# sina-behnam/RTSDS

Measured on AMD Instinct MI355X. Metric: images/sec/node (train step) + inference FPS@1024x512, BiSeNet 19-cls, higher is better.
Workload: dtype bf16; 1 GPU; configs[1]: BiSeNet-R18 seg-only train step (train.py:65-113); model=BiSeNet-ResNet18, global_batch=8, per_gpu_batch=8, image=3x512x1024, num_classes=19, parallelism=dp1

## Files before the change

include/rtsds_hip.h:

```cpp
#ifndef RTSDS_HIP_H
#define RTSDS_HIP_H
#include <stddef.h>
#include <stdint.h>
#ifdef __cplusplus
extern "C" {
#endif

enum { RTSDS_F32 = 0, RTSDS_BF16 = 1, RTSDS_F16 = 2  };
enum {
  RTSDS_OK = 0,
  RTSDS_ERR_SHAPE = 1,
  RTSDS_ERR_UNSUPPORTED = 2,
  RTSDS_ERR_LAUNCH = 3,
  RTSDS_ERR_WORKSPACE = 4
};
enum { RTSDS_ACT_NONE = 0, RTSDS_ACT_RELU = 1, RTSDS_ACT_LEAKY = 2, RTSDS_ACT_SIGMOID = 3 };
#define RTSDS_ACCUMULATE 0x100
#define RTSDS_INPUT_PADDED 0x400
#define RTSDS_WEIGHT_PACKED 0x800

typedef struct {
  int n, h, w, c;
  int ho, wo, k;
  int kh, kw;
// ... 188 lines not shown
int rtsds_ce_weighted_bwd(const void* x, long sn, long sc, long shw, const int64_t* target,
                          const float* weight, const float* grad_loss, const float* count, void* dx,
                          int n, long hw, int c, int ignore_index, int dtype, void* stream);
int rtsds_bce_fwd(const float* x, const float* target, float* loss, int n, void* stream);
int rtsds_bce_bwd(const float* x, const float* target, const float* grad_loss, float* dx, int n,
                  void* stream);

int rtsds_adam_step(float* param, const void* grad, float* exp_avg, float* exp_avg_sq,
                    void* bf16_shadow, long n, float lr, float beta1, float beta2, float eps,
                    float weight_decay, int step, float grad_scale, int grad_dtype, void* stream);

int rtsds_adam_step_dev(float* param, const void* grad, float* exp_avg, float* exp_avg_sq,
                        void* bf16_shadow, long n, const float* hyper, float beta1, float beta2,
                        float eps, float weight_decay, float grad_scale, int grad_dtype, void* stream);

int rtsds_sgd_step(float* param, const void* grad, float* momentum_buf, void* bf16_shadow,
                   long n, const float* hyper, float lr, float momentum, float dampening,
                   float weight_decay, int nesterov, int first, float grad_scale, int grad_dtype, void* stream);

int rtsds_ema_step(float* teacher, const float* student, void* teacher_bf16_shadow, long n, float w,
                   void* stream);
int rtsds_ema_many(int count, float* const* teacher, const float* const* student, const long* numel,
                   float w, void* stream);

int rtsds_argmax(const void* x, long sn, long sc, long shw, int64_t* out, const int64_t* target,
                 unsigned long long* correct, int n, long hw, int c, int dtype, void* stream);
int rtsds_confusion(const int64_t* label, const int64_t* pred, unsigned long long* hist, long total,
                    int nc, void* stream);

#define RTSDS_UPCE_SET_CORRECT 2
// ... 126 lines not shown
                        void* pooled, void* hid, void* att, void* r, int ldr, int n, long hw, int c, int dtype,
                        void* stream);
int rtsds_ffm_att_bwd(const void* dr, const void* f, const void* a, const void* h, const void* p, const void* w1,
                      const void* w2, float* dw1, float* db1, float* dw2, float* db2, void* dp, int n, long hw, int c,
                      int accumulate, int dtype, void* ws, size_t ws_bytes, void* stream);
int rtsds_bn_bwd_ffm(const void* dr, const void* att, const void* dpooled, int n, long hw, const void* x, void* dx,
                     float* dgamma, float* dbeta, int c, const float* gamma, const float* beta, const float* save_mean,
                     const float* save_invstd, int training, int act, int accumulate_params, int dtype, void* ws,
                     size_t ws_bytes, void* stream);

size_t rtsds_label_stats_workspace(int n, int c);
int rtsds_label_stats(const int64_t* label, int n, int h, int w, int c, int ignore_index,
                      unsigned long long* count, unsigned long long* support, void* ws, size_t ws_bytes,
                      void* stream);

#define RTSDS_ABI_VERSION 28
int rtsds_abi_version(void);

#ifdef __cplusplus
}
#endif
#endif
```

rtsds_amd/_lib.py:

```python
import ctypes
import os

import torch

_HERE = os.path.dirname(os.path.abspath(__file__))
DEFAULT_LIB_PATH = os.path.join(_HERE, "librtsds_hip.so")
ABI_VERSION = 28
LIB_PATH = os.environ.get("RTSDS_LIB") or DEFAULT_LIB_PATH

F32, BF16 = 0, 1
ACT_NONE, ACT_RELU, ACT_LEAKY, ACT_SIGMOID = 0, 1, 2, 3
ACCUMULATE = 0x100
INPUT_PADDED = 0x400
WEIGHT_PACKED = 0x800
UPCE_SET_CORRECT = 2
ERRORS = {1: "bad shape", 2: "unsupported configuration", 3: "HIP launch failure", 4: "workspace too small"}

c_int, c_long, c_float, c_double, c_size_t, c_void_p = (ctypes.c_int, ctypes.c_long, ctypes.c_float, ctypes.c_double,
                                                        ctypes.c_size_t, ctypes.c_void_p)


class ConvDesc(ctypes.Structure):
    _fields_ = [(n, c_int) for n in ("n", "h", "w", "c", "ho", "wo", "k", "kh", "kw", "sh", "sw",
                                     "ph", "pw", "dh", "dw", "dtype")]
# ... 102 lines not shown
    "rtsds_softmax_fwd": (c_int, [P, c_long, c_long, c_long, P, c_int, c_int, c_long, c_int, c_int, P]),
    "rtsds_softmax_bwd": (c_int, [P, P, c_int, P, c_long, c_long, c_long, c_int, c_long, c_int, c_int,
                                  P]),
    "rtsds_ce_workspace": (c_size_t, []),
    "rtsds_ce_fwd": (c_int, [P, c_long, c_long, c_long, P, P, c_int, c_long, c_int, c_int, c_int, P,
                             c_size_t, P]),
    "rtsds_ce_bwd": (c_int, [P, c_long, c_long, c_long, P, P, P, P, c_int, c_long, c_int, c_int, c_int,
                             P]),
    "rtsds_ce_weighted_fwd": (c_int, [P, c_long, c_long, c_long, P, P, P, c_int, c_long, c_int, c_int, c_int, P,
                                      c_size_t, P]),
    "rtsds_ce_weighted_bwd": (c_int, [P, c_long, c_long, c_long, P, P, P, P, P, c_int, c_long, c_int, c_int, c_int,
                                      P]),
    "rtsds_bce_fwd": (c_int, [P, P, P, c_int, P]),
    "rtsds_bce_bwd": (c_int, [P, P, P, P, c_int, P]),
    "rtsds_adam_step_dev": (c_int, [P, P, P, P, P, c_long, P, c_float, c_float, c_float, c_float, c_float, c_int, P]),
    "rtsds_upsoftmax_fwd": (c_int, [P, P, c_int, c_int, c_int, c_int, c_int, c_int, c_float, c_float, c_int, c_int, P]),
    "rtsds_upsoftmax_bwd_workspace": (c_size_t, [c_int, c_int, c_int, c_int, c_int, c_int]),
    "rtsds_upsoftmax_bwd": (c_int, [P, c_int, P, c_int, P, c_int, c_int, c_int, c_int, c_int, c_int, c_float, c_float,
                                    c_int, P, c_size_t, P]),
    "rtsds_upselfinfo_fwd": (c_int, [P, P, c_int, c_int, c_int, c_int, c_int, c_int, c_float, c_float, c_int, c_int, P]),
    "rtsds_upselfinfo_bwd_workspace": (c_size_t, [c_int, c_int, c_int, c_int, c_int, c_int]),
    "rtsds_upselfinfo_bwd": (c_int, [P, c_int, P, P, c_int, c_int, c_int, c_int, c_int, c_int, c_float, c_float, c_int, P,
                                     c_size_t, P]),
    "rtsds_upsoftmax_acc": (c_int, [P, P, P, c_int, c_int, c_int, c_int, c_int, c_int, c_float, c_float, c_int, c_int,
                                    c_int, P]),
    "rtsds_conf_hist": (c_int, [P, P, P, P, c_long, c_int, c_int, c_float, P]),
    "rtsds_pseudo_select": (c_int, [P, P, P, P, c_long, c_int, c_int, P]),
    "rtsds_upsample_pseudo": (c_int, [P, P, P, P, P] + [c_int] * 6 + [c_float, c_float, c_int, c_int, c_int, P]),
    "rtsds_upsample_paint": (c_int, [P, P, P, P, P, P] + [c_int] * 6 + [c_float, c_float, c_int, c_int, P]),
    "rtsds_slide_paint": (c_int, [P, ctypes.POINTER(c_int), c_int, P, P, P, P, P, P] + [c_int] * 8 +
# ... 88 lines not shown
```

rtsds_amd/csrc/conv_wgrad.hip:

```cpp
#include "conv_host.h"

template <int V>
__global__ void __launch_bounds__(256) split_reduce_kernel(const float* __restrict__ part, float* __restrict__ out, int nv,
                                                            int cv, FastDiv fcv, int cp, long slab, int splits, int accumulate) {
  __shared__ float red[4][64][V];
  const int lane = threadIdx.x & 63, sg = threadIdx.x >> 6;
  for (int i0 = blockIdx.x * 64; i0 < nv; i0 += gridDim.x * 64) {
    const int i = i0 + lane;
    const bool ok = i < nv;
    const int rt = (int)fdiv((uint32_t)(ok ? i : 0), fcv);
    const long src = (long)rt * cp + (long)((ok ? i : 0) - rt * cv) * V;
    float s[V];
#pragma unroll
    for (int e = 0; e < V; ++e) s[e] = 0.f;
    for (int q = sg; ok && q < splits; q += 32) {
      float t[8][V];
#pragma unroll
      for (int u = 0; u < 8; ++u) {
        const long off = (long)min(q + 4 * u, splits - 1) * slab + src;
        if constexpr (V == 4) {
          const f32x4 v = *(const f32x4*)(part + off);
#pragma unroll
          for (int e = 0; e < V; ++e) t[u][e] = v[e];
        } else {
// ... 203 lines not shown

static const int kReduceBatch = 16;
struct ReduceBatch {
  rtsds_split_reduce_desc d[kReduceBatch];
  int blk0[kReduceBatch];
  int n;
};
__global__ void __launch_bounds__(256) split_reduce_many_kernel(const ReduceBatch b) {
  __shared__ float red[4][64][4];
  int si = 0;
  for (int i = 1; i < b.n; ++i)
    if (b.blk0[i] <= (int)blockIdx.x) si = i;
  const rtsds_split_reduce_desc& q = b.d[si];
  const int lane = threadIdx.x & 63, sg = threadIdx.x >> 6;
  const int i = ((int)blockIdx.x - b.blk0[si]) * 64 + lane;
  const bool ok = i < q.nv;
  const int rt = (ok ? i : 0) / q.cv;
  const long src = (long)rt * q.cp + (long)((ok ? i : 0) - rt * q.cv) * 4;
  float s[4] = {0.f, 0.f, 0.f, 0.f};
  for (int g = sg; ok && g < q.splits; g += 32) {
    float t[8][4];
#pragma unroll
    for (int u = 0; u < 8; ++u) {
      const f32x4 v = *(const f32x4*)(q.slab + (long)min(g + 4 * u, q.splits - 1) * q.slab_stride + src);
#pragma unroll
      for (int e = 0; e < 4; ++e) t[u][e] = v[e];
    }
#pragma unroll
    for (int u = 0; u < 8; ++u)
      if (g + 4 * u < q.splits)
#pragma unroll
        for (int e = 0; e < 4; ++e) s[e] += t[u][e];
  }
#pragma unroll
  for (int e = 0; e < 4; ++e) red[sg][lane][e] = s[e];
  __syncthreads();
  if (sg == 0 && ok) {
    float* o = q.dw + (long)i * 4;
#pragma unroll
    for (int e = 0; e < 4; ++e) {
      const float t = (red[0][lane][e] + red[1][lane][e]) + (red[2][lane][e] + red[3][lane][e]);
      o[e] = q.accumulate ? o[e] + t : t;
    }
  }
}
extern "C" int rtsds_split_reduce_many(int n, const rtsds_split_reduce_desc* descs, void* stream) {
  if (n < 0 || (n && !descs)) return RTSDS_ERR_SHAPE;
  for (int i0 = 0; i0 < n; i0 += kReduceBatch) {
    ReduceBatch b;
    b.n = 0;
    int blocks = 0;
    for (int i = i0; i < n && b.n < kReduceBatch; ++i) {
      if (descs[i].nv <= 0) continue;
      if (descs[i].cv <= 0 || descs[i].splits <= 0 || !descs[i].slab || !descs[i].dw) return RTSDS_ERR_SHAPE;
      b.d[b.n] = descs[i];
      b.blk0[b.n] = blocks;
      blocks += (descs[i].nv + 63) / 64;
      ++b.n;
// ... 192 lines not shown
```

rtsds_amd/csrc/optim.hip:

```cpp
#include "ew_common.h"

template <typename GT>
__global__ void adam_kernel(float* __restrict__ p, const GT* __restrict__ g, float* __restrict__ m, float* __restrict__ v,
                            bf16* __restrict__ shadow, long n, float lr, float b1, float b2, float eps, float wd, float bc1,
                            float bc2_sqrt, float gscale) {
  const float step = lr / bc1;
  GRID_STRIDE(i, n) {
    float gi = to_f(g[i]) * gscale;
    float pi = p[i];
    if (wd != 0.f) gi = fmaf(wd, pi, gi);
    float mi = m[i], vi = v[i];
    mi = fmaf(1.f - b1, gi - mi, mi);
    vi = fmaf(b2, vi, (1.f - b2) * gi * gi);
    const float den = sqrtf(vi) / bc2_sqrt + eps;
    pi -= step * (mi / den);
    m[i] = mi;
    v[i] = vi;
    p[i] = pi;
    if (shadow) shadow[i] = (bf16)pi;
  }
}
template <typename GT>
__global__ void adam_dev_kernel(float* __restrict__ p, const GT* __restrict__ g, float* __restrict__ m, float* __restrict__ v,
                                bf16* __restrict__ shadow, long n, const float* __restrict__ hyper, float b1, float b2, float eps,
                                float wd, float gscale) {
  const float lr = hyper[0], bc1 = hyper[1], bc2_sqrt = hyper[2];
  const float step = lr / bc1;
  GRID_STRIDE(i, n) {
    float gi = to_f(g[i]) * gscale;
    float pi = p[i];
    if (wd != 0.f) gi = fmaf(wd, pi, gi);
    float mi = m[i], vi = v[i];
    mi = fmaf(1.f - b1, gi - mi, mi);
    vi = fmaf(b2, vi, (1.f - b2) * gi * gi);
    const float den = sqrtf(vi) / bc2_sqrt + eps;
    pi -= step * (mi / den);
    m[i] = mi;
    v[i] = vi;
    p[i] = pi;
    if (shadow) shadow[i] = (bf16)pi;
  }
}
#define DISPATCH_GRAD(gd, ...)                                               \
  do {                                                                       \
    if ((gd) == RTSDS_F32) { typedef float GT; __VA_ARGS__; }                \
    else if ((gd) == RTSDS_BF16) { typedef bf16 GT; __VA_ARGS__; }           \
    else if ((gd) == RTSDS_F16) { typedef f16 GT; __VA_ARGS__; }             \
    else return RTSDS_ERR_UNSUPPORTED;                                       \
  } while (0)
extern "C" int rtsds_adam_step_dev(float* param, const void* grad, float* exp_avg, float* exp_avg_sq, void* bf16_shadow,
                                   long n, const float* hyper, float beta1, float beta2, float eps, float weight_decay,
                                   float grad_scale, int grad_dtype, void* stream) {
  if (n <= 0 || !hyper) return RTSDS_ERR_SHAPE;
  DISPATCH_GRAD(grad_dtype, hipLaunchKernelGGL(adam_dev_kernel<GT>, dim3(ew_blocks(n, 256, 4096)), dim3(256), 0,
                                               (hipStream_t)stream, param, (const GT*)grad, exp_avg, exp_avg_sq,
                                               (bf16*)bf16_shadow, n, hyper, beta1, beta2, eps, weight_decay, grad_scale));
  RET_LAUNCH();
}

extern "C" int rtsds_adam_step(float* param, const void* grad, float* exp_avg, float* exp_avg_sq, void* bf16_shadow, long n, float lr,
                               float beta1, float beta2, float eps, float weight_decay, int step, float grad_scale, int grad_dtype,
                               void* stream) {
  if (n <= 0 || step <= 0) return RTSDS_ERR_SHAPE;
  const double bc1 = 1.0 - pow((double)beta1, step), bc2 = 1.0 - pow((double)beta2, step);
  DISPATCH_GRAD(grad_dtype, hipLaunchKernelGGL(adam_kernel<GT>, dim3(ew_blocks(n, 256, 4096)), dim3(256), 0, (hipStream_t)stream,
                                               param, (const GT*)grad, exp_avg, exp_avg_sq, (bf16*)bf16_shadow, n, lr, beta1, beta2,
                                               eps, weight_decay, (float)bc1, (float)sqrt(bc2), grad_scale));
  RET_LAUNCH();
}

template <typename GT>
__global__ void sgd_kernel(float* __restrict__ p, const GT* __restrict__ g, float* __restrict__ buf,
                           bf16* __restrict__ shadow, long n, const float* __restrict__ hyper, float lr, float momentum,
                           float dampening, float wd, int nesterov, int first, float gscale) {
// ... 95 lines not shown
```

rtsds_amd/functional.py:

```python
import ctypes

import numpy as np
import torch

from ._lib import (ACT_RELU, ACT_SIGMOID, INPUT_PADDED, UPCE_SET_CORRECT, WEIGHT_PACKED, BnParams, ConvDesc,
                   SplitReduceDesc, lib)
from .runtime import (CL, bump_params_epoch, collective, dcode, dp_world, empty_nhwc, nhwc, params_epoch,
                      register_fold, require_hip, side_enabled, side_fork, stream, workspace)

_P = lambda t: None if t is None else t.data_ptr()

CONV_PROFILE = None


def _conv_flops(d):
    return 2.0 * d.n * d.ho * d.wo * d.k * d.c * d.kh * d.kw


class _Timed:
    def __init__(self, d, tag="fwd"):
        self.d, self.tag = d, tag

    def __enter__(self):
        if CONV_PROFILE is not None:
# ... 124 lines not shown


def _join_add(join, g):
    if join is None:
        return g
    if join.buf is not None:
        if join.first:
            join.buf.add_(g)
            return join.put(join.buf)
        g.add_(join.buf)
    return join.put(g)


DEFER_WGRAD_REDUCE = True
_deferred = []


def flush_wgrad_reduce():
    global _deferred
    items, _deferred = _deferred, []
    if not items:
        return
    cur = torch.cuda.current_stream(items[0][1].device)
    for st in {it[2] for it in items}:
        if st != cur:
            cur.wait_stream(st)
    batch, seen = [], set()
    for desc, _ws, _st in items + [(None, None, None)]:
        if desc is None or desc.dw in seen or len(batch) == 16:
            if batch:
                arr = (SplitReduceDesc * len(batch))(*batch)
                lib.rtsds_split_reduce_many(len(batch), arr, cur.cuda_stream)
            batch, seen = [], set()
        if desc is not None:
            batch.append(desc)
            seen.add(desc.dw)
    for _desc, ws, st in items:
        if st != cur:
            ws.record_stream(cur)


def _wgrad_into_arena(d, x, g, sinks, xflag, ws):
    if DEFER_WGRAD_REDUCE and CONV_PROFILE is None and x.dtype == torch.bfloat16:
        pend = SplitReduceDesc()
        lib.rtsds_conv2d_wgrad_deferred(ctypes.byref(d), _P(x), _P(g), _P(sinks[0]), _P(sinks[1]), 1 | xflag,
                                        _P(ws), ws.numel(), ctypes.byref(pend), stream())
        if pend.nv > 0:
            _deferred.append((pend, ws, torch.cuda.current_stream(ws.device)))
            torch.autograd.Variable._execution_engine.queue_callback(flush_wgrad_reduce)
        return
    with _Timed(d, "wgrad"):
        lib.rtsds_conv2d_wgrad(ctypes.byref(d), _P(x), _P(g), _P(sinks[0]), _P(sinks[1]), 1 | xflag,
                               _P(ws), ws.numel(), stream())


class ConvFn(torch.autograd.Function):

    @staticmethod
    def forward(ctx, x, weight, bias, wq, stride, padding, dilation, act, stats, join=None, fold=(0, False),
                bn_link=None, wg_link=None):
        require_hip(x, weight)
        k, _, kh, kw = weight.shape
        padded = hasattr(x, "_rt_cpad") and is_padded_input(x, _conv_desc(x, k, kh, kw, stride, padding, dilation))
        if not padded:
# ... 69 lines not shown
                                                   _P(bsm), _P(bsi), bact | wpk, _P(part), _P(ws), ws.numel(), stream())
                    link.part, link.nrb = part, tiles
                elif ctx.in_act:
                    lib.rtsds_conv2d_dgrad_act(ctypes.byref(d), _P(g), _P(wd), _P(dx), _P(x), ctx.in_act | wpk,
                                               _P(ws), ws.numel(), stream())
                else:
                    lib.rtsds_conv2d_dgrad(ctypes.byref(d), _P(g), _P(wd), _P(dx), (1 if acc else 0) | wpk, _P(ws),
                                           ws.numel(), stream())
            if join is not None:
                dx = join.put(dx)
        if (ctx.needs_input_grad[1] or ctx.needs_input_grad[2]) and not wg_side:
            weight, bias = ctx.params
            sinks = _sinks(weight, bias if ctx.needs_input_grad[2] else None) if ctx.needs_input_grad[1] else None
            ws = workspace(lib.rtsds_conv2d_wgrad_workspace(ctypes.byref(d)), x.device)
            if sinks is not None:
                _wgrad_into_arena(d, x, g, sinks, ctx.xflag, ws)
                dw = None
                db = None
            else:
                dw = torch.empty((d.k, d.c, d.kh, d.kw), dtype=torch.float32, device=x.device,
                                 memory_format=CL)
                db = torch.empty(d.k, dtype=torch.float32, device=x.device) if ctx.has_bias else None
                with _Timed(d, "wgrad"):
                    lib.rtsds_conv2d_wgrad(ctypes.byref(d), _P(x), _P(g), _P(dw), _P(db), ctx.xflag, _P(ws),
                                                  ws.numel(), stream())
                if not ctx.needs_input_grad[1]:
                    dw = None
        return dx, dw, db, None, None, None, None, None, None, None, None, None, None


def _img_bn_wgrad(d, x, g, bx, coef, act, weight, xflag):
    ws = workspace(lib.rtsds_imgconv_bn_wgrad_workspace(ctypes.byref(d)), x.device)
    sinks = _sinks(weight)
    if sinks is not None and DEFER_WGRAD_REDUCE and CONV_PROFILE is None:
        pend = SplitReduceDesc()
        lib.rtsds_imgconv_bn_wgrad_deferred(ctypes.byref(d), _P(x), _P(g), _P(bx), _P(coef), act, _P(sinks[0]),
                                            1 | xflag, _P(ws), ws.numel(), ctypes.byref(pend), stream())
        _deferred.append((pend, ws, torch.cuda.current_stream(ws.device)))
        torch.autograd.Variable._execution_engine.queue_callback(flush_wgrad_reduce)
        return None
    dw = sinks[0] if sinks is not None else torch.empty((d.k, d.c, d.kh, d.kw), dtype=torch.float32,
                                                         device=x.device, memory_format=CL)
    with _Timed(d, "wgrad"):
        lib.rtsds_imgconv_bn_wgrad(ctypes.byref(d), _P(x), _P(g), _P(bx), _P(coef), act, _P(dw),
                                   (1 if sinks is not None else 0) | xflag, _P(ws), ws.numel(), stream())
    return None if sinks is not None else dw


def conv2d(x, weight, bias, wq, stride=(1, 1), padding=(0, 0), dilation=(1, 1), act=0, bn_stats=False,
           join=None, in_act=0, fold_out=False, bn_link=None, wg_link=None):
    stats = nrb = None
    if bn_stats and act == 0:
        n, _, h, w = x.shape
        k, _, kh, kw = weight.shape
# ... 1873 lines not shown
```

rtsds_amd/optim.py:

```python
import ctypes
import warnings

import torch
import torch.distributed as dist

from ._lib import ConvDesc, lib
from .runtime import bump_params_epoch, collective, dp_world, stream


_ALLREDUCE = {"dtype": torch.float32}


def set_allreduce_dtype(dtype):
    if dtype not in (torch.float32, torch.float16, torch.bfloat16):
        raise ValueError("all-reduce dtype must be float32, float16 or bfloat16")
    _ALLREDUCE["dtype"] = dtype


_DCODE = {torch.float32: 0, torch.bfloat16: 1, torch.float16: 2}


def wire_active():
    return _ALLREDUCE["dtype"] != torch.float32 and dp_world() > 1 and dist.is_available() and dist.is_initialized()


def _to_wire(buffers, wires):
    if _ALLREDUCE["dtype"] == torch.float32:
        return [(b, None) for b in buffers]
    if wires is None:
        return [(b.to(_ALLREDUCE["dtype"]), b) for b in buffers]
    out = []
    for b, w in zip(buffers, wires):
        lib.rtsds_cast(b.data_ptr(), 0, w.data_ptr(), _DCODE[w.dtype], b.numel(), stream())
        out.append((w, None))
# ... 30 lines not shown
    pending, pairs = [], _to_wire(buffers, wires)
    for t, _ in pairs:
        collective(lambda t=t: pending.append(dist.all_reduce(t, async_op=True)))

    def wait_all():
        for h in pending:
            h.wait()
        pending.clear()

    def finish():
        collective(wait_all)
        for t, back in pairs:
            if back is not None:
                back.copy_(t)
    return finish


class _Arena:

    def __init__(self, params, second=True):
        dev = params[0].device
        self.params = params
        self.offsets = []
        total = 0
        for p in params:
            if p.dtype != torch.float32 or not p.is_cuda:
                raise RuntimeError("rtsds_amd.optim: fp32 HIP parameters required")
            if not (p.is_contiguous() or p.is_contiguous(memory_format=torch.channels_last)):
                p.data = p.data.contiguous()
            self.offsets.append(total)
            total += (p.numel() + 63) // 64 * 64
        self.total = total
        self.flat = torch.zeros(total, dtype=torch.float32, device=dev)
        self.gflat = torch.zeros(total, dtype=torch.float32, device=dev)
        self.m = torch.zeros(total, dtype=torch.float32, device=dev)
        self.v = torch.zeros(total, dtype=torch.float32, device=dev) if second else None
        self.shadow = torch.empty(total, dtype=torch.bfloat16, device=dev)
        self.gwire = None
        self.steps = [0] * len(params)
        self.touched = [False] * len(params)
        self.gen = [0] * len(params)
        self.reduced = None
        self.dpacks = []
        with torch.no_grad():
            for i, p in enumerate(params):
                off, n = self.offsets[i], p.numel()
                view = self.flat[off:off + n].as_strided(p.shape, p.stride())
                view.copy_(p.data)
                p.data = view
                p.grad = self.gflat[off:off + n].as_strided(p.shape, p.stride())
        lib.rtsds_cast(self.flat.data_ptr(), 0, self.shadow.data_ptr(), 1, total, stream())
        for i, p in enumerate(params):
            off, n = self.offsets[i], p.numel()
            if p.dim() == 4:
                p._rt_shadow = self.shadow[off:off + n].as_strided(p.shape, p.stride())
                p._rt_shadow_key = (p.data_ptr(), p._version)
            p._rt_arena = (self, i)
            if p.requires_grad:
                p.register_post_accumulate_grad_hook(self._hook(i))

    def wire(self):
        dt = _ALLREDUCE["dtype"]
        if self.gwire is None or self.gwire.dtype != dt:
            self.gwire = torch.zeros(self.total, dtype=dt, device=self.gflat.device)
        return self.gwire

    def reduced_grad(self):
        return self.gwire.float() if wire_active() and self.gwire is not None else self.gflat

    def _hook(self, i):
        def mark(_p):
            self._check_open(i)
            self.touched[i] = True
            self.gen[i] = _GEN[0]
        return mark

    def _check_open(self, i):
        if self.reduced is not None and self.reduced[i]:
            raise RuntimeError(f"rtsds_amd.optim: a gradient of parameter {i} ({tuple(self.params[i].shape)}) arrived "
                               "after its all-reduce started (start_grad_allreduce(partial=True)): the backward cut "
                               "must separate the parameters of the two phases")

    def repack(self):
        live = [p for p in self.dpacks if p._rt_dpack.arena is self and getattr(p, "_rt_shadow", None) is not None]
        if not live:
            return
        n = len(live)
        descs = (ConvDesc * n)(*[p._rt_dpack.desc for p in live])
        src = (ctypes.c_void_p * n)(*[p._rt_shadow.data_ptr() for p in live])
        dst = (ctypes.c_void_p * n)(*[p._rt_dpack.buf.data_ptr() for p in live])
        lib.rtsds_conv2d_dgrad_pack_many(n, descs, src, dst, stream())
        for p in live:
            p._rt_dpack.valid = p._rt_shadow_key

    def sink(self, i):
        if not self.grad_ptr_ok(i):
            return None
        self._check_open(i)
        self.touched[i] = True
        self.gen[i] = _GEN[0]
        return self.params[i].grad

    def grad_ptr_ok(self, i):
        p = self.params[i]
        return p.grad is not None and p.grad.data_ptr() == self.gflat.data_ptr() + 4 * self.offsets[i]

    def rebind_grad(self, i):
        p = self.params[i]
        off, n = self.offsets[i], p.numel()
        view = self.gflat[off:off + n].as_strided(p.shape, p.stride())
        if p.grad is not None:
            view.copy_(p.grad)
        p.grad = view


class _FlatOptimizer(torch.optim.Optimizer):

    _STATE = ()
    _NAME = "optimizer"

    def __init__(self, params, defaults):
        super().__init__(params, defaults)
        self._arenas = None
        self._warned = False
        self._graph = False
        self._capturing = False
        self._runs = None
        self._hyper = None
        self._ring = [[None, None] for _ in range(8)]
        self._ring_pos = 0
        self._finish = []
        self._reduced = None

    def _ensure(self):
        if self._arenas is None:
            self._arenas = [_Arena(sorted(g["params"], key=lambda p: not p.requires_grad),
                                   second=len(self._STATE) > 1) for g in self.param_groups]
            self._import_state()
        return self._arenas

    def arenas(self):
        return self._ensure()

    def _view(self, a, i, attr):
        p, off = a.params[i], a.offsets[i]
        return getattr(a, attr)[off:off + p.numel()].as_strided(p.shape, p.stride())

# ... 26 lines not shown
                for i, p in enumerate(a.params):
                    if a.steps[i] > 0:
                        self.state[p] = self._exported(a, i)
        try:
            return super().state_dict()
        finally:
            if self._arenas is not None:
                self.state.clear()

    def load_state_dict(self, state_dict):
        super().load_state_dict(state_dict)
        if self._arenas is not None:
            self._import_state()

    def zero_grad(self, set_to_none=True):
        for a in self._ensure():
            a.gflat.zero_()
            for i in range(len(a.params)):
                a.touched[i] = False
                if not a.grad_ptr_ok(i):
                    a.rebind_grad(i)
                    a.gflat[a.offsets[i]:a.offsets[i] + a.params[i].numel()].zero_()

    def _fix_grads(self, arenas):
        for a in arenas:
            for i in range(len(a.params)):
                if a.touched[i] and not a.grad_ptr_ok(i):
                    if not self._warned:
                        warnings.warn(f"rtsds_amd.{self._NAME}: gradient left the arena; copying back")
                        self._warned = True
                    a.rebind_grad(i)

    @staticmethod
    def _ranges(a, idx):
        out = []
        for i in idx:
            lo, hi = a.offsets[i], a.offsets[i] + a.params[i].numel()
            if out and out[-1][2] == i - 1:
                out[-1] = (out[-1][0], hi, i)
            else:
                out.append((lo, hi, i))
        return [(lo, hi) for lo, hi, _ in out]

    @torch.no_grad()
    def start_grad_allreduce(self, partial=False, since=None):
        if not _OVERLAP["on"] or dp_world() <= 1 or not (dist.is_available() and dist.is_initialized()):
            return
        arenas = self._ensure()
        self._fix_grads(arenas)
        if self._reduced is None:
            self._reduced = [[False] * len(a.params) for a in arenas]
            for a, red in zip(arenas, self._reduced):
                a.reduced = red
        bufs, wires = [], []
        for a, red in zip(arenas, self._reduced):
            idx = [i for i in range(len(a.params)) if not red[i] and
                   (not partial or (a.touched[i] and (since is None or a.gen[i] >= since)))]
            for i in idx:
                red[i] = True
            rng = self._ranges(a, idx)
            bufs += [a.gflat[lo:hi] for lo, hi in rng]
            if wire_active():
                wires += [a.wire()[lo:hi] for lo, hi in rng]
# ... 20 lines not shown
        else:
            self._fix_grads(arenas)
            gscale = allreduce_flat([a.gflat for a in arenas], [a.wire() for a in arenas] if wire_active() else None)
        runs = []
        for gi, a in enumerate(arenas):
            i, n = 0, len(a.params)
            while i < n:
                if not a.touched[i]:
                    i += 1
                    continue
                j = i
                while j + 1 < n and a.touched[j + 1] and a.steps[j + 1] == a.steps[i]:
                    j += 1
                runs.append((gi, i, j))
                i = j + 1
        if self._capturing:
            if runs != self._runs or self._hyper is None:
                raise RuntimeError(f"rtsds_amd.{self._NAME}: step structure changed under graph capture")
        else:
            self._runs = runs
            if self._graph:
                self.stage_hyper()
        for r, (gi, i, j) in enumerate(runs):
            g, a = self.param_groups[gi], arenas[gi]
            lo = a.offsets[i]
            hi = a.offsets[j] + a.params[j].numel()
            hyper = self._hyper.data_ptr() + 12 * r if self._graph else None
            self._launch(g, a, lo, hi, a.steps[i] + 1, hyper, gscale)
            for k in range(i, j + 1):
                a.steps[k] += 1
        for a in arenas:
            if a.shadow is not None:
                a.repack()
        return loss

    def set_graph_mode(self, on=True):
        self._graph = bool(on)

    def stage_hyper(self):
        runs = self._runs or []
        arenas = self._ensure()
        flat = []
        for gi, i, _ in runs:
            flat.extend(self._hyper3(self.param_groups[gi], arenas[gi].steps[i] + 1))
        n = max(1, len(flat))
# ... 45 lines not shown
        if amsgrad:
            raise NotImplementedError("rtsds_amd.optim.Adam: amsgrad")
        super().__init__(params, dict(lr=lr, betas=betas, eps=eps, weight_decay=weight_decay))

    def _launch(self, g, a, lo, hi, t, hyper, gscale):
        b1, b2 = g["betas"]
        gp, gd = _grad(a, lo)
        ptrs = _ptrs(a, lo, hi, "flat") + (gp,) + _ptrs(a, lo, hi, "m", "v") + (a.shadow.data_ptr() + 2 * lo, hi - lo)
        if hyper is not None:
            lib.rtsds_adam_step_dev(*ptrs, hyper, float(b1), float(b2), float(g["eps"]),
                                    float(g["weight_decay"]), gscale, gd, stream())
        else:
            lib.rtsds_adam_step(*ptrs, float(g["lr"]), float(b1), float(b2), float(g["eps"]),
                                float(g["weight_decay"]), t, gscale, gd, stream())

    def _hyper3(self, g, t):
        b1, b2 = (float(torch.tensor(b, dtype=torch.float32)) for b in g["betas"])
        return [float(g["lr"]), 1.0 - b1 ** t, (1.0 - b2 ** t) ** 0.5]


class SGD(_FlatOptimizer):

    _STATE = (("m", "momentum_buffer"),)
    _NAME = "SGD"

    def __init__(self, params, lr=1e-3, momentum=0, dampening=0, weight_decay=0, nesterov=False,
                 maximize=False):
        if maximize:
            raise NotImplementedError("rtsds_amd.optim.SGD: maximize")
        if nesterov and (momentum <= 0 or dampening != 0):
# ... 25 lines not shown
```

rtsds_amd/train.py:

```python
import contextlib

import torch

from . import functional as F
from . import losses, utils
from .optim import begin_grad_phase
from .runtime import branch_stream, branches_enabled, branches_serial, collect_cuts, dp_world
from .callbacks import Callback
from .validation import val_GTA5

try:
    from tqdm import tqdm
except ImportError:
    def tqdm(it, **_):
        return it


def _host_values(tensors):
    t = torch.stack([x.double().reshape(()) for x in tensors])
    if dp_world() > 1:
        import torch.distributed as dist
        dist.all_reduce(t)
    return t.tolist()

# ... 25 lines not shown
    key = (t.device, t.dtype, tuple(t.shape))
    one = _ONES.get(key)
    if one is None:
        one = _ONES[key] = torch.ones_like(t)
    return one


def _backward(loss, optimizer, cuts, since=None):
    loss.backward(_one(loss))
    for x, xd in reversed(cuts or []):
        optimizer.start_grad_allreduce(partial=True, since=since)
        if xd.grad is not None:
            torch.autograd.backward([x], [xd.grad])


def seg_step(model, criterion, optimizer, inputs, targets):
    optimizer.zero_grad()
    split = dp_world() > 1 and hasattr(optimizer, "start_grad_allreduce")
    with collect_cuts(split) as cuts:
        fused = _fused_heads(model, criterion, inputs)
        if fused is None:
            outs = _unpack(model(inputs))
    if fused is not None and fused[1] is not None:
        correct = torch.empty(1, dtype=torch.int64, device=fused[0][0].device)
        loss = F.upsample_cross_entropy(fused[0], targets, fused[1], criterion.ignore_index, correct, set_correct=True,
                                        weight=criterion.weight)
        _backward(loss, optimizer, cuts)
        optimizer.step()
        return loss.detach(), correct
    if fused is not None:
        outs = list(fused[0]) + [None] * (3 - len(fused[0]))
        main_output, aux1, aux2 = outs[:3]
    else:
        main_output, aux1, aux2 = outs
    loss = criterion(main_output, targets)
    if aux1 is not None:
        loss = loss + criterion(aux1, targets)
    if aux2 is not None:
        loss = loss + criterion(aux2, targets)
    _backward(loss, optimizer, cuts)
    optimizer.step()
    correct = torch.zeros(1, dtype=torch.int64, device=main_output.device)
    F.argmax_channels(main_output.detach(), targets, correct, want_map=False)
    return loss.detach(), correct


def train(epoch: int, model: torch.nn.Module, train_loader, criterion: torch.nn.Module,
          optimizer: torch.optim.Optimizer, init_lr: float, max_iter: int, power: float = 0.9,
          lr_decay_iter: float = 1.0, device: str = "cuda", callbacks: list = []):
    for cb in callbacks:
        cb.on_train_begin()
    model.train()
    running_loss, correct, total = 0.0, 0, 0
    for batch_idx, (inputs, targets) in tqdm(enumerate(train_loader), total=len(train_loader),
# ... 351 lines not shown
```

Before: 1855 images/s.

## Fuse deferred split-K weight-grad reduction into Adam step and zero only dirty grad ranges

Deferred wgrad split-slab reductions are handed to the optimizer, and a new kernel reduces each slab and applies the Adam update in one pass. This avoids writing reduced gradients to memory and reading them back, and removes the separate reduce launches. zero_grad now clears only the gradient ranges that were actually written, through a range-zeroing kernel, using dirty/lazy tracking per parameter. In exchange, the grad-state bookkeeping becomes more complex, which raises the risk of stale gradients if the tracking is wrong.

Result: faster. 1882 images/s, median of 6 (+1.5%).

```diff
diff --git a/include/rtsds_hip.h b/include/rtsds_hip.h
--- a/include/rtsds_hip.h
+++ b/include/rtsds_hip.h
@@ -226,6 +226,13 @@
                         void* bf16_shadow, long n, const float* hyper, float beta1, float beta2,
                         float eps, float weight_decay, float grad_scale, int grad_dtype, void* stream);
 
+#define RTSDS_SLAB_KEEP_GRAD 2
+int rtsds_adam_step_slabs(float* param, float* grad, float* exp_avg, float* exp_avg_sq, void* bf16_shadow,
+                          long n, const float* hyper, float beta1, float beta2, float eps,
+                          float weight_decay, float grad_scale, int grad_dtype, int n_descs,
+                          const rtsds_split_reduce_desc* descs, int max_descs, void* stream);
+int rtsds_zero_ranges(float* buf, int count, const long* lo, const long* hi, void* stream);
+
 int rtsds_sgd_step(float* param, const void* grad, float* momentum_buf, void* bf16_shadow,
                    long n, const float* hyper, float lr, float momentum, float dampening,
                    float weight_decay, int nesterov, int first, float grad_scale, int grad_dtype, void* stream);
@@ -382,7 +389,7 @@
                       unsigned long long* count, unsigned long long* support, void* ws, size_t ws_bytes,
                       void* stream);
 
-#define RTSDS_ABI_VERSION 28
+#define RTSDS_ABI_VERSION 29
 int rtsds_abi_version(void);
 
 #ifdef __cplusplus
diff --git a/rtsds_amd/_lib.py b/rtsds_amd/_lib.py
--- a/rtsds_amd/_lib.py
+++ b/rtsds_amd/_lib.py
@@ -5,7 +5,7 @@
 
 _HERE = os.path.dirname(os.path.abspath(__file__))
 DEFAULT_LIB_PATH = os.path.join(_HERE, "librtsds_hip.so")
-ABI_VERSION = 28
+ABI_VERSION = 29
 LIB_PATH = os.environ.get("RTSDS_LIB") or DEFAULT_LIB_PATH
 
 F32, BF16 = 0, 1
@@ -140,6 +140,9 @@
     "rtsds_bce_fwd": (c_int, [P, P, P, c_int, P]),
     "rtsds_bce_bwd": (c_int, [P, P, P, P, c_int, P]),
     "rtsds_adam_step_dev": (c_int, [P, P, P, P, P, c_long, P, c_float, c_float, c_float, c_float, c_float, c_int, P]),
+    "rtsds_adam_step_slabs": (c_int, [P, P, P, P, P, c_long, P, c_float, c_float, c_float, c_float, c_float, c_int, c_int,
+                                      ctypes.POINTER(SplitReduceDesc), c_int, P]),
+    "rtsds_zero_ranges": (c_int, [P, c_int, ctypes.POINTER(c_long), ctypes.POINTER(c_long), P]),
     "rtsds_upsoftmax_fwd": (c_int, [P, P, c_int, c_int, c_int, c_int, c_int, c_int, c_float, c_float, c_int, c_int, P]),
     "rtsds_upsoftmax_bwd_workspace": (c_size_t, [c_int, c_int, c_int, c_int, c_int, c_int]),
     "rtsds_upsoftmax_bwd": (c_int, [P, c_int, P, c_int, P, c_int, c_int, c_int, c_int, c_int, c_int, c_float, c_float,
diff --git a/rtsds_amd/csrc/conv_wgrad.hip b/rtsds_amd/csrc/conv_wgrad.hip
--- a/rtsds_amd/csrc/conv_wgrad.hip
+++ b/rtsds_amd/csrc/conv_wgrad.hip
@@ -1,4 +1,5 @@
 #include "conv_host.h"
+#include "split_reduce_dev.h"
 
 template <int V>
 __global__ void __launch_bounds__(256) split_reduce_kernel(const float* __restrict__ part, float* __restrict__ out, int nv,
@@ -241,34 +242,12 @@
   const rtsds_split_reduce_desc& q = b.d[si];
   const int lane = threadIdx.x & 63, sg = threadIdx.x >> 6;
   const int i = ((int)blockIdx.x - b.blk0[si]) * 64 + lane;
-  const bool ok = i < q.nv;
-  const int rt = (ok ? i : 0) / q.cv;
-  const long src = (long)rt * q.cp + (long)((ok ? i : 0) - rt * q.cv) * 4;
-  float s[4] = {0.f, 0.f, 0.f, 0.f};
-  for (int g = sg; ok && g < q.splits; g += 32) {
-    float t[8][4];
-#pragma unroll
-    for (int u = 0; u < 8; ++u) {
-      const f32x4 v = *(const f32x4*)(q.slab + (long)min(g + 4 * u, q.splits - 1) * q.slab_stride + src);
-#pragma unroll
-      for (int e = 0; e < 4; ++e) t[u][e] = v[e];
-    }
-#pragma unroll
-    for (int u = 0; u < 8; ++u)
-      if (g + 4 * u < q.splits)
-#pragma unroll
-        for (int e = 0; e < 4; ++e) s[e] += t[u][e];
-  }
-#pragma unroll
-  for (int e = 0; e < 4; ++e) red[sg][lane][e] = s[e];
-  __syncthreads();
-  if (sg == 0 && ok) {
+  float t[4];
+  split_reduce_block(q, i, red, t);
+  if (sg == 0 && i < q.nv) {
     float* o = q.dw + (long)i * 4;
 #pragma unroll
-    for (int e = 0; e < 4; ++e) {
-      const float t = (red[0][lane][e] + red[1][lane][e]) + (red[2][lane][e] + red[3][lane][e]);
-      o[e] = q.accumulate ? o[e] + t : t;
-    }
+    for (int e = 0; e < 4; ++e) o[e] = q.accumulate ? o[e] + t[e] : t[e];
   }
 }
 extern "C" int rtsds_split_reduce_many(int n, const rtsds_split_reduce_desc* descs, void* stream) {
diff --git a/rtsds_amd/csrc/optim.hip b/rtsds_amd/csrc/optim.hip
--- a/rtsds_amd/csrc/optim.hip
+++ b/rtsds_amd/csrc/optim.hip
@@ -1,19 +1,22 @@
 #include "ew_common.h"
-
+#include "split_reduce_dev.h"
+
+RT_DEV void adam_elem(float& pi, float gi, float& mi, float& vi, float step, float b1, float b2, float eps, float wd,
+                      float bc2_sqrt) {
+  if (wd != 0.f) gi = fmaf(wd, pi, gi);
+  mi = fmaf(1.f - b1, gi - mi, mi);
+  vi = fmaf(b2, vi, (1.f - b2) * gi * gi);
+  const float den = sqrtf(vi) / bc2_sqrt + eps;
+  pi -= step * (mi / den);
+}
 template <typename GT>
 __global__ void adam_kernel(float* __restrict__ p, const GT* __restrict__ g, float* __restrict__ m, float* __restrict__ v,
                             bf16* __restrict__ shadow, long n, float lr, float b1, float b2, float eps, float wd, float bc1,
                             float bc2_sqrt, float gscale) {
   const float step = lr / bc1;
   GRID_STRIDE(i, n) {
-    float gi = to_f(g[i]) * gscale;
-    float pi = p[i];
-    if (wd != 0.f) gi = fmaf(wd, pi, gi);
-    float mi = m[i], vi = v[i];
-    mi = fmaf(1.f - b1, gi - mi, mi);
-    vi = fmaf(b2, vi, (1.f - b2) * gi * gi);
-    const float den = sqrtf(vi) / bc2_sqrt + eps;
-    pi -= step * (mi / den);
+    float pi = p[i], mi = m[i], vi = v[i];
+    adam_elem(pi, to_f(g[i]) * gscale, mi, vi, step, b1, b2, eps, wd, bc2_sqrt);
     m[i] = mi;
     v[i] = vi;
     p[i] = pi;
@@ -27,14 +30,8 @@
   const float lr = hyper[0], bc1 = hyper[1], bc2_sqrt = hyper[2];
   const float step = lr / bc1;
   GRID_STRIDE(i, n) {
-    float gi = to_f(g[i]) * gscale;
-    float pi = p[i];
-    if (wd != 0.f) gi = fmaf(wd, pi, gi);
-    float mi = m[i], vi = v[i];
-    mi = fmaf(1.f - b1, gi - mi, mi);
-    vi = fmaf(b2, vi, (1.f - b2) * gi * gi);
-    const float den = sqrtf(vi) / bc2_sqrt + eps;
-    pi -= step * (mi / den);
+    float pi = p[i], mi = m[i], vi = v[i];
+    adam_elem(pi, to_f(g[i]) * gscale, mi, vi, step, b1, b2, eps, wd, bc2_sqrt);
     m[i] = mi;
     v[i] = vi;
     p[i] = pi;
@@ -58,6 +55,170 @@
   RET_LAUNCH();
 }
 
+static const int kAdamSlabMax = 56;
+static const int kAdamPlainChunk = 4096;
+struct AdamSlabArgs {
+  rtsds_split_reduce_desc d[kAdamSlabMax];
+  int blk0[kAdamSlabMax];
+  int gap_lo[kAdamSlabMax + 1], gap_hi[kAdamSlabMax + 1];
+  int gblk0[kAdamSlabMax + 1];
+  int n, ngaps, slab_blocks;
+};
+static_assert(sizeof(AdamSlabArgs) <= 3840, "AdamSlabArgs must fit the kernel argument segment with the pointers");
+__global__ void __launch_bounds__(256) adam_slabs_kernel(const AdamSlabArgs a, float* __restrict__ p, float* __restrict__ g,
+                                                         float* __restrict__ m, float* __restrict__ v, bf16* __restrict__ shadow,
+                                                         const float* __restrict__ hyper, float b1, float b2, float eps, float wd,
+                                                         float gscale) {
+  __shared__ float red[4][64][4];
+  const float lr = hyper[0], bc1 = hyper[1], bc2_sqrt = hyper[2];
+  const float step = lr / bc1;
+  const int b = blockIdx.x;
+  if (b < a.slab_blocks) {
+    int si = 0;
+    for (int i = 1; i < a.n; ++i)
+      if (a.blk0[i] <= b) si = i;
+    const rtsds_split_reduce_desc& q = a.d[si];
+    const int lane = threadIdx.x & 63, sg = threadIdx.x >> 6;
+    const int i = (b - a.blk0[si]) * 64 + lane;
+    float t[4];
+    split_reduce_block(q, i, red, t);
+    if (sg != 0 || i >= q.nv) return;
+    const long off = (q.dw - g) + (long)i * 4;
+    if (q.accumulate & 1) {
+      const f32x4 o = *(const f32x4*)(g + off);
+#pragma unroll
+      for (int e = 0; e < 4; ++e) t[e] = o[e] + t[e];
+    }
+    if (q.accumulate & RTSDS_SLAB_KEEP_GRAD) *(f32x4*)(g + off) = f32x4{t[0], t[1], t[2], t[3]};
+    f32x4 pv = *(const f32x4*)(p + off), mv = *(const f32x4*)(m + off), vv = *(const f32x4*)(v + off);
+    bf16x4 h;
+#pragma unroll
+    for (int e = 0; e < 4; ++e) {
+      float pi = pv[e], mi = mv[e], vi = vv[e];
+      adam_elem(pi, t[e] * gscale, mi, vi, step, b1, b2, eps, wd, bc2_sqrt);
+      pv[e] = pi; mv[e] = mi; vv[e] = vi;
+      h[e] = (bf16)pi;
+    }
+    *(f32x4*)(m + off) = mv;
+    *(f32x4*)(v + off) = vv;
+    *(f32x4*)(p + off) = pv;
+    if (shadow) *(bf16x4*)(shadow + off) = h;
+    return;
+  }
+  const int pb = b - a.slab_blocks;
+  int gi = 0;
+  for (int i = 1; i < a.ngaps; ++i)
+    if (a.gblk0[i] <= pb) gi = i;
+  const long lo = a.gap_lo[gi] + (long)(pb - a.gblk0[gi]) * kAdamPlainChunk;
+  const long hi = min((long)a.gap_hi[gi], lo + kAdamPlainChunk);
+  for (long e0 = lo + 4 * (long)threadIdx.x; e0 < hi; e0 += 4 * 256) {
+    if (e0 + 4 <= hi) {
+      const f32x4 gv = *(const f32x4*)(g + e0);
+      f32x4 pv = *(const f32x4*)(p + e0), mv = *(const f32x4*)(m + e0), vv = *(const f32x4*)(v + e0);
+      bf16x4 h;
+#pragma unroll
+      for (int e = 0; e < 4; ++e) {
+        float pi = pv[e], mi = mv[e], vi = vv[e];
+        adam_elem(pi, gv[e] * gscale, mi, vi, step, b1, b2, eps, wd, bc2_sqrt);
+        pv[e] = pi; mv[e] = mi; vv[e] = vi;
+        h[e] = (bf16)pi;
+      }
+      *(f32x4*)(m + e0) = mv;
+      *(f32x4*)(v + e0) = vv;
+      *(f32x4*)(p + e0) = pv;
+      if (shadow) *(bf16x4*)(shadow + e0) = h;
+    } else {
+      for (long i = e0; i < hi; ++i) {
+        float pi = p[i], mi = m[i], vi = v[i];
+        adam_elem(pi, g[i] * gscale, mi, vi, step, b1, b2, eps, wd, bc2_sqrt);
+        m[i] = mi;
+        v[i] = vi;
+        p[i] = pi;
+        if (shadow) shadow[i] = (bf16)pi;
+      }
+    }
+  }
+}
+extern "C" int rtsds_adam_step_slabs(float* param, float* grad, float* exp_avg, float* exp_avg_sq, void* bf16_shadow, long n,
+                                     const float* hyper, float beta1, float beta2, float eps, float weight_decay,
+                                     float grad_scale, int grad_dtype, int n_descs, const rtsds_split_reduce_desc* descs,
+                                     int max_descs, void* stream) {
+  if (n <= 0 || !hyper || !param || !grad || !exp_avg || !exp_avg_sq || n_descs < 0 || (n_descs && !descs) || max_descs < 0)
+    return RTSDS_ERR_SHAPE;
+  const int cap = max_descs ? std::min(max_descs, kAdamSlabMax) : kAdamSlabMax;
+  if (grad_dtype != RTSDS_F32 || n_descs > cap || n >= INT_MAX - kAdamPlainChunk) return RTSDS_ERR_UNSUPPORTED;
+  if ((((uintptr_t)param | (uintptr_t)grad | (uintptr_t)exp_avg | (uintptr_t)exp_avg_sq) & 15) || ((uintptr_t)bf16_shadow & 7))
+    return RTSDS_ERR_UNSUPPORTED;
+  AdamSlabArgs a;
+  a.n = n_descs;
+  a.ngaps = 0;
+  long sblocks = 0, pblocks = 0, at = 0;
+  auto gap = [&](long lo, long hi) {
+    if (hi <= lo) return;
+    a.gap_lo[a.ngaps] = (int)lo;
+    a.gap_hi[a.ngaps] = (int)hi;
+    a.gblk0[a.ngaps] = (int)pblocks;
+    pblocks += (hi - lo + kAdamPlainChunk - 1) / kAdamPlainChunk;
+    ++a.ngaps;
+  };
+  for (int i = 0; i < n_descs; ++i) {
+    const rtsds_split_reduce_desc& q = descs[i];
+    if (q.nv <= 0 || q.cv <= 0 || q.splits <= 0 || !q.slab || !q.dw) return RTSDS_ERR_SHAPE;
+    if (((uintptr_t)q.dw & 15) || ((uintptr_t)q.slab & 15) || (q.slab_stride & 3) || (q.cp & 3)) return RTSDS_ERR_UNSUPPORTED;
+    const long lo = q.dw - grad, hi = lo + 4L * q.nv;
+    if (q.dw < grad || lo < at || hi > n) return RTSDS_ERR_SHAPE;
+    a.d[i] = q;
+    a.blk0[i] = (int)sblocks;
+    sblocks += (q.nv + 63) / 64;
+    gap(at, lo);
+    at = hi;
+  }
+  gap(at, n);
+  if (sblocks + pblocks > INT_MAX) return RTSDS_ERR_UNSUPPORTED;
+  a.slab_blocks = (int)sblocks;
+  hipLaunchKernelGGL(adam_slabs_kernel, dim3((unsigned)(sblocks + pblocks)), dim3(256), 0, (hipStream_t)stream, a, param, grad,
+                     exp_avg, exp_avg_sq, (bf16*)bf16_shadow, hyper, beta1, beta2, eps, weight_decay, grad_scale);
+  RET_LAUNCH();
+}
+
+static const int kZeroRanges = 128, kZeroChunk = 4096;
+struct ZeroRangeArgs {
+  long lo[kZeroRanges];
+  int len[kZeroRanges], blk0[kZeroRanges];
+  int n;
+};
+__global__ void __launch_bounds__(256) zero_ranges_kernel(const ZeroRangeArgs a, float* __restrict__ buf) {
+  int ri = 0;
+  for (int i = 1; i < a.n; ++i)
+    if (a.blk0[i] <= (int)blockIdx.x) ri = i;
+  const int r0 = ((int)blockIdx.x - a.blk0[ri]) * kZeroChunk, r1 = min(a.len[ri], r0 + kZeroChunk);
+  float* o = buf + a.lo[ri] + r0;
+  const int n = r1 - r0, nv = ((uintptr_t)o & 15) == 0 ? n >> 2 : 0;
+  for (int i = threadIdx.x; i < nv; i += 256) ((f32x4*)o)[i] = f32x4{0.f, 0.f, 0.f, 0.f};
+  for (int i = 4 * nv + threadIdx.x; i < n; i += 256) o[i] = 0.f;
+}
+extern "C" int rtsds_zero_ranges(float* buf, int count, const long* lo, const long* hi, void* stream) {
+  if (count < 0 || (count && (!buf || !lo || !hi))) return RTSDS_ERR_SHAPE;
+  for (int i = 0; i < count; ++i)
+    if (lo[i] < 0 || hi[i] < lo[i] || hi[i] - lo[i] > INT_MAX - kZeroChunk) return RTSDS_ERR_SHAPE;
+  for (int i0 = 0; i0 < count; i0 += kZeroRanges) {
+    ZeroRangeArgs a;
+    a.n = 0;
+    long blocks = 0;
+    for (int i = i0; i < count && i < i0 + kZeroRanges; ++i) {
+      if (hi[i] == lo[i]) continue;
+      a.lo[a.n] = lo[i];
+      a.len[a.n] = (int)(hi[i] - lo[i]);
+      a.blk0[a.n] = (int)blocks;
+      blocks += (hi[i] - lo[i] + kZeroChunk - 1) / kZeroChunk;
+      ++a.n;
+    }
+    if (blocks > INT_MAX) return RTSDS_ERR_UNSUPPORTED;
+    if (a.n) hipLaunchKernelGGL(zero_ranges_kernel, dim3((unsigned)blocks), dim3(256), 0, (hipStream_t)stream, a, buf);
+  }
+  RET_LAUNCH();
+}
+
 extern "C" int rtsds_adam_step(float* param, const void* grad, float* exp_avg, float* exp_avg_sq, void* bf16_shadow, long n, float lr,
                                float beta1, float beta2, float eps, float weight_decay, int step, float grad_scale, int grad_dtype,
                                void* stream) {
diff --git a/rtsds_amd/csrc/split_reduce_dev.h b/rtsds_amd/csrc/split_reduce_dev.h
--- /dev/null
+++ b/rtsds_amd/csrc/split_reduce_dev.h
@@ -0,0 +1,31 @@
+#pragma once
+#include "common.h"
+
+RT_DEV void split_reduce_block(const rtsds_split_reduce_desc& q, int i, float (*red)[64][4], float* t) {
+  const int lane = threadIdx.x & 63, sg = threadIdx.x >> 6;
+  const bool ok = i < q.nv;
+  const int rt = (ok ? i : 0) / q.cv;
+  const long src = (long)rt * q.cp + (long)((ok ? i : 0) - rt * q.cv) * 4;
+  float s[4] = {0.f, 0.f, 0.f, 0.f};
+  for (int g = sg; ok && g < q.splits; g += 32) {
+    float v8[8][4];
+#pragma unroll
+    for (int u = 0; u < 8; ++u) {
+      const f32x4 v = *(const f32x4*)(q.slab + (long)min(g + 4 * u, q.splits - 1) * q.slab_stride + src);
+#pragma unroll
+      for (int e = 0; e < 4; ++e) v8[u][e] = v[e];
+    }
+#pragma unroll
+    for (int u = 0; u < 8; ++u)
+      if (g + 4 * u < q.splits)
+#pragma unroll
+        for (int e = 0; e < 4; ++e) s[e] += v8[u][e];
+  }
+#pragma unroll
+  for (int e = 0; e < 4; ++e) red[sg][lane][e] = s[e];
+  __syncthreads();
+  if (sg == 0 && ok) {
+#pragma unroll
+    for (int e = 0; e < 4; ++e) t[e] = (red[0][lane][e] + red[1][lane][e]) + (red[2][lane][e] + red[3][lane][e]);
+  }
+}
diff --git a/rtsds_amd/functional.py b/rtsds_amd/functional.py
--- a/rtsds_amd/functional.py
+++ b/rtsds_amd/functional.py
@@ -162,19 +162,17 @@
 
 DEFER_WGRAD_REDUCE = True
 _deferred = []
-
-
-def flush_wgrad_reduce():
-    global _deferred
-    items, _deferred = _deferred, []
-    if not items:
-        return
-    cur = torch.cuda.current_stream(items[0][1].device)
-    for st in {it[2] for it in items}:
-        if st != cur:
-            cur.wait_stream(st)
+FUSE_REDUCE_ADAM = True
+_fuse_into = [None]
+
+
+def fuse_wgrad_reduce_into(optimizer):
+    _fuse_into[0] = optimizer if FUSE_REDUCE_ADAM and DEFER_WGRAD_REDUCE else None
+
+
+def reduce_wgrads_now(items, cur):
     batch, seen = [], set()
-    for desc, _ws, _st in items + [(None, None, None)]:
+    for desc, *_ in list(items) + [(None,)]:
         if desc is None or desc.dw in seen or len(batch) == 16:
             if batch:
                 arr = (SplitReduceDesc * len(batch))(*batch)
@@ -183,19 +181,46 @@
         if desc is not None:
             batch.append(desc)
             seen.add(desc.dw)
-    for _desc, ws, st in items:
+    for _desc, _ws, _st, weight, _keep in items:
+        arena, i = weight._rt_arena
+        arena.dirty[i] = True
+
+
+def flush_wgrad_reduce():
+    global _deferred
+    items, _deferred = _deferred, []
+    owner, _fuse_into[0] = _fuse_into[0], None
+    if not items:
+        return
+    cur = torch.cuda.current_stream(items[0][1].device)
+    for st in {it[2] for it in items}:
+        if st != cur:
+            cur.wait_stream(st)
+    mine = []
+    if owner is not None and FUSE_REDUCE_ADAM:
+        own = owner.arenas()
+        mine = [it for it in items if any(it[3]._rt_arena[0] is a for a in own)]
+        owner.take_wgrad_reduces(mine)
+    reduce_wgrads_now([it for it in items if not any(it is m for m in mine)], cur)
+    for _desc, ws, st, *_ in items:
         if st != cur:
             ws.record_stream(cur)
 
 
-def _wgrad_into_arena(d, x, g, sinks, xflag, ws):
+def _defer(pend, ws, weight, keep=False):
+    arena, i = weight._rt_arena
+    arena.sink_unwritten(i)
+    _deferred.append((pend, ws, torch.cuda.current_stream(ws.device), weight, keep))
+    torch.autograd.Variable._execution_engine.queue_callback(flush_wgrad_reduce)
+
+
+def _wgrad_into_arena(d, x, g, sinks, xflag, ws, weight):
     if DEFER_WGRAD_REDUCE and CONV_PROFILE is None and x.dtype == torch.bfloat16:
         pend = SplitReduceDesc()
         lib.rtsds_conv2d_wgrad_deferred(ctypes.byref(d), _P(x), _P(g), _P(sinks[0]), _P(sinks[1]), 1 | xflag,
                                         _P(ws), ws.numel(), ctypes.byref(pend), stream())
         if pend.nv > 0:
-            _deferred.append((pend, ws, torch.cuda.current_stream(ws.device)))
-            torch.autograd.Variable._execution_engine.queue_callback(flush_wgrad_reduce)
+            _defer(pend, ws, weight)
         return
     with _Timed(d, "wgrad"):
         lib.rtsds_conv2d_wgrad(ctypes.byref(d), _P(x), _P(g), _P(sinks[0]), _P(sinks[1]), 1 | xflag,
@@ -295,7 +320,7 @@
             sinks = _sinks(weight, bias if ctx.needs_input_grad[2] else None) if ctx.needs_input_grad[1] else None
             ws = workspace(lib.rtsds_conv2d_wgrad_workspace(ctypes.byref(d)), x.device)
             if sinks is not None:
-                _wgrad_into_arena(d, x, g, sinks, ctx.xflag, ws)
+                _wgrad_into_arena(d, x, g, sinks, ctx.xflag, ws, weight)
                 dw = None
                 db = None
             else:
@@ -317,8 +342,7 @@
         pend = SplitReduceDesc()
         lib.rtsds_imgconv_bn_wgrad_deferred(ctypes.byref(d), _P(x), _P(g), _P(bx), _P(coef), act, _P(sinks[0]),
                                             1 | xflag, _P(ws), ws.numel(), ctypes.byref(pend), stream())
-        _deferred.append((pend, ws, torch.cuda.current_stream(ws.device)))
-        torch.autograd.Variable._execution_engine.queue_callback(flush_wgrad_reduce)
+        _defer(pend, ws, weight, keep=True)
         return None
     dw = sinks[0] if sinks is not None else torch.empty((d.k, d.c, d.kh, d.kw), dtype=torch.float32,
                                                          device=x.device, memory_format=CL)
diff --git a/rtsds_amd/optim.py b/rtsds_amd/optim.py
--- a/rtsds_amd/optim.py
+++ b/rtsds_amd/optim.py
@@ -4,7 +4,7 @@
 import torch
 import torch.distributed as dist
 
-from ._lib import ConvDesc, lib
+from ._lib import ERRORS, ConvDesc, SplitReduceDesc, lib, load
 from .runtime import bump_params_epoch, collective, dp_world, stream
 
 
@@ -18,6 +18,7 @@
 
 
 _DCODE = {torch.float32: 0, torch.bfloat16: 1, torch.float16: 2}
+SLAB_KEEP_GRAD = 2
 
 
 def wire_active():
@@ -78,6 +79,31 @@
             if back is not None:
                 back.copy_(t)
     return finish
+
+
+def zero_plan(offsets, total, need):
+    out = []
+    for i, off in enumerate(offsets):
+        if not need[i]:
+            continue
+        end = offsets[i + 1] if i + 1 < len(offsets) else total
+        if out and out[-1][1] == off:
+            out[-1] = (out[-1][0], end)
+        else:
+            out.append((off, end))
+    return out
+
+
+def slab_plan(lo, hi, targets):
+    order = sorted(range(len(targets)), key=lambda k: targets[k][0])
+    holes, at = [], lo
+    for k in order:
+        off, n = targets[k]
+        if n <= 0 or n % 4 or off % 4 or off < at or off + n > hi:
+            return None
+        holes.append((off, off + n))
+        at = off + n
+    return order, holes
 
 
 class _Arena:
@@ -103,6 +129,9 @@
         self.gwire = None
         self.steps = [0] * len(params)
         self.touched = [False] * len(params)
+        self.dirty = [False] * len(params)
+        self.lazy = [False] * len(params)
+        self._was_dirty = [False] * len(params)
         self.gen = [0] * len(params)
         self.reduced = None
         self.dpacks = []
@@ -113,6 +142,7 @@
                 view.copy_(p.data)
                 p.data = view
                 p.grad = self.gflat[off:off + n].as_strided(p.shape, p.stride())
+        self._gver = self.gflat._version
         lib.rtsds_cast(self.flat.data_ptr(), 0, self.shadow.data_ptr(), 1, total, stream())
         for i, p in enumerate(params):
             off, n = self.offsets[i], p.numel()
@@ -136,6 +166,9 @@
         def mark(_p):
             self._check_open(i)
             self.touched[i] = True
+            if self.gflat._version != self._gver:
+                self._gver = self.gflat._version
+                self.dirty[i] = True
             self.gen[i] = _GEN[0]
         return mark
 
@@ -162,8 +195,13 @@
             return None
         self._check_open(i)
         self.touched[i] = True
+        self._was_dirty[i], self.dirty[i] = self.dirty[i], True
         self.gen[i] = _GEN[0]
         return self.params[i].grad
+
+    def sink_unwritten(self, i):
+        self.dirty[i] = self._was_dirty[i]
+        self.lazy[i] = True
 
     def grad_ptr_ok(self, i):
         p = self.params[i]
@@ -175,6 +213,7 @@
         view = self.gflat[off:off + n].as_strided(p.shape, p.stride())
         if p.grad is not None:
             view.copy_(p.grad)
+            self.dirty[i] = True
         p.grad = view
 
 
@@ -195,6 +234,7 @@
         self._ring_pos = 0
         self._finish = []
         self._reduced = None
+        self._pending = []
 
     def _ensure(self):
         if self._arenas is None:
@@ -251,13 +291,50 @@
             self._import_state()
 
     def zero_grad(self, set_to_none=True):
+        self._pending = []
         for a in self._ensure():
-            a.gflat.zero_()
-            for i in range(len(a.params)):
-                a.touched[i] = False
+            n = len(a.params)
+            for i in range(n):
                 if not a.grad_ptr_ok(i):
                     a.rebind_grad(i)
-                    a.gflat[a.offsets[i]:a.offsets[i] + a.params[i].numel()].zero_()
+            need = [a.dirty[i] or (a.touched[i] and not a.lazy[i]) for i in range(n)]
+            rng = zero_plan(a.offsets, a.total, need)
+            if rng == [(0, a.total)]:
+                a.gflat.zero_()
+            elif rng:
+                lo = (ctypes.c_long * len(rng))(*[r[0] for r in rng])
+                hi = (ctypes.c_long * len(rng))(*[r[1] for r in rng])
+                lib.rtsds_zero_ranges(a.gflat.data_ptr(), len(rng), lo, hi, stream())
+            for i in range(n):
+                a.touched[i] = a.dirty[i] = a.lazy[i] = False
+            a._gver = a.gflat._version
+
+    fuses_wgrad_reduce = False
+    SLAB_MAX_DESCS = 0
+
+    def take_wgrad_reduces(self, items):
+        self._pending = self._pending + list(items)
+
+    @torch.no_grad()
+    def materialize_grads(self):
+        items, self._pending = self._pending, []
+        if items:
+            from .functional import reduce_wgrads_now
+            reduce_wgrads_now(items, torch.cuda.current_stream(items[0][1].device))
+
+    def _can_fuse(self, arenas, gscale):
+        if not self.fuses_wgrad_reduce or dp_world() > 1 or wire_active() or gscale != 1.0:
+            return False
+        seen = set()
+        for desc, _ws, _st, weight, _keep in self._pending:
+            a, i = weight._rt_arena
+            if desc.dw in seen or not a.touched[i] or not a.grad_ptr_ok(i) or not any(a is b for b in arenas):
+                return False
+            seen.add(desc.dw)
+        return True
+
+    def _launch_slabs(self, g, a, lo, hi, hyper, gscale, items):
+        return False
 
     def _fix_grads(self, arenas):
         for a in arenas:
@@ -284,6 +361,7 @@
         if not _OVERLAP["on"] or dp_world() <= 1 or not (dist.is_available() and dist.is_initialized()):
             return
         arenas = self._ensure()
+        self.materialize_grads()
         self._fix_grads(arenas)
         if self._reduced is None:
             self._reduced = [[False] * len(a.params) for a in arenas]
@@ -334,21 +412,32 @@
                     j += 1
                 runs.append((gi, i, j))
                 i = j + 1
+        pend = self._pending
+        if pend and not self._can_fuse(arenas, gscale):
+            self.materialize_grads()
+            pend = []
         if self._capturing:
             if runs != self._runs or self._hyper is None:
                 raise RuntimeError(f"rtsds_amd.{self._NAME}: step structure changed under graph capture")
         else:
             self._runs = runs
-            if self._graph:
+            if self._graph or pend:
                 self.stage_hyper()
         for r, (gi, i, j) in enumerate(runs):
             g, a = self.param_groups[gi], arenas[gi]
             lo = a.offsets[i]
             hi = a.offsets[j] + a.params[j].numel()
-            hyper = self._hyper.data_ptr() + 12 * r if self._graph else None
-            self._launch(g, a, lo, hi, a.steps[i] + 1, hyper, gscale)
+            mine = [it for it in pend if it[3]._rt_arena[0] is a and i <= it[3]._rt_arena[1] <= j]
+            if mine and not self._launch_slabs(g, a, lo, hi, self._hyper.data_ptr() + 12 * r, gscale, mine):
+                from .functional import reduce_wgrads_now
+                reduce_wgrads_now(mine, torch.cuda.current_stream(a.flat.device))
+                mine = []
+            if not mine:
+                hyper = self._hyper.data_ptr() + 12 * r if self._graph else None
+                self._launch(g, a, lo, hi, a.steps[i] + 1, hyper, gscale)
             for k in range(i, j + 1):
                 a.steps[k] += 1
+        self._pending = []
         for a in arenas:
             if a.shadow is not None:
                 a.repack()
@@ -424,6 +513,32 @@
             lib.rtsds_adam_step(*ptrs, float(g["lr"]), float(b1), float(b2), float(g["eps"]),
                                 float(g["weight_decay"]), t, gscale, gd, stream())
 
+    fuses_wgrad_reduce = True
+
+    def _launch_slabs(self, g, a, lo, hi, hyper, gscale, items):
+        base = a.gflat.data_ptr()
+        plan = slab_plan(lo, hi, [((it[0].dw - base) // 4, 4 * it[0].nv) for it in items])
+        if plan is None:
+            return False
+        descs = (SplitReduceDesc * len(items))()
+        for k, src in enumerate(plan[0]):
+            desc, _ws, _st, weight, keep = items[src]
+            i = weight._rt_arena[1]
+            ctypes.memmove(ctypes.byref(descs[k]), ctypes.byref(desc), ctypes.sizeof(SplitReduceDesc))
+            descs[k].accumulate = (1 if a.dirty[i] else 0) | (SLAB_KEEP_GRAD if keep else 0)
+        b1, b2 = g["betas"]
+        rc = load().rtsds_adam_step_slabs(*_ptrs(a, lo, hi, "flat", "gflat", "m", "v"), a.shadow.data_ptr() + 2 * lo, hi - lo,
+                                          hyper, float(b1), float(b2), float(g["eps"]), float(g["weight_decay"]), gscale, 0,
+                                          len(items), descs, int(self.SLAB_MAX_DESCS), stream())
+        if rc == 2:
+            return False
+        if rc != 0:
+            raise RuntimeError(f"rtsds_amd: rtsds_adam_step_slabs failed: {ERRORS.get(rc, rc)}")
+        for _desc, _ws, _st, weight, keep in items:
+            if keep:
+                a.dirty[weight._rt_arena[1]] = True
+        return True
+
     def _hyper3(self, g, t):
         b1, b2 = (float(torch.tensor(b, dtype=torch.float32)) for b in g["betas"])
         return [float(g["lr"]), 1.0 - b1 ** t, (1.0 - b2 ** t) ** 0.5]
diff --git a/rtsds_amd/train.py b/rtsds_amd/train.py
--- a/rtsds_amd/train.py
+++ b/rtsds_amd/train.py
@@ -63,6 +63,11 @@
             torch.autograd.backward([x], [xd.grad])
 
 
+def _fuse_reduce(optimizer):
+    ok = dp_world() == 1 and getattr(optimizer, "fuses_wgrad_reduce", False)
+    F.fuse_wgrad_reduce_into(optimizer if ok else None)
+
+
 def seg_step(model, criterion, optimizer, inputs, targets):
     optimizer.zero_grad()
     split = dp_world() > 1 and hasattr(optimizer, "start_grad_allreduce")
@@ -74,6 +79,7 @@
         correct = torch.empty(1, dtype=torch.int64, device=fused[0][0].device)
         loss = F.upsample_cross_entropy(fused[0], targets, fused[1], criterion.ignore_index, correct, set_correct=True,
                                         weight=criterion.weight)
+        _fuse_reduce(optimizer)
         _backward(loss, optimizer, cuts)
         optimizer.step()
         return loss.detach(), correct
@@ -87,6 +93,7 @@
         loss = loss + criterion(aux1, targets)
     if aux2 is not None:
         loss = loss + criterion(aux2, targets)
+    _fuse_reduce(optimizer)
     _backward(loss, optimizer, cuts)
     optimizer.step()
     correct = torch.zeros(1, dtype=torch.int64, device=main_output.device)
```
